# wrchen530/batrack

Measured on AMD Instinct MI355X. Metric: BA iterations/s on 64-KF/128k-edge graph, higher is better.
Workload: dtype f32

## Files before the change

### batrack_amd/csrc/ba_solve.hip

```cpp
#include <hip/hip_runtime.h>

#include "ba_kernels.hpp"
#include "ba_update.hpp"
#include "ba_wave.hpp"

namespace bt {

__device__ inline bool chol6_inv(float *Ablk, float *Linv) {
    float L[6][6];
#pragma unroll
    for (int r = 0; r < 6; ++r)
#pragma unroll
        for (int c = 0; c < 6; ++c) L[r][c] = c <= r ? Ablk[6*r + c] : 0.0f;
    bool ok = true;
#pragma unroll
    for (int c = 0; c < 6; ++c) {
        float s = L[c][c];
#pragma unroll
        for (int k = 0; k < c; ++k) s -= L[c][k] * L[c][k];
        if (!(s > 0.0f)) ok = false;
        const float l = sqrtf(s), il = 1.0f / l;
        L[c][c] = l;
#pragma unroll
        for (int r = c + 1; r < 6; ++r) {
// ... 467 lines not shown
#pragma unroll
                    for (int k = 1; k < kMaxLevelCols; ++k) q += item >= rows_before[k] ? 1 : 0;
                    const int rw = item - (q == 0 ? 0 : q == 1 ? rows_before[1] : q == 2 ? rows_before[2] : rows_before[3]);
                    const int4 ma = q == 0 ? mA0 : q == 1 ? mA1 : q == 2 ? mA2 : mA3;
                    const int j = ma.x, dpos = ma.y, cnt = ma.z;
                    T L[21];
                    const T *dblk = Lw + (size_t)dpos * 36;
#pragma unroll
                    for (int r = 0; r < 6; ++r) {
                        T row[6];
                        load_row6(dblk + 6 * r, row);
#pragma unroll
                        for (int c = 0; c <= r; ++c) L[BT_LT(r, c)] = row[c];
                    }
                    T *p = rw < cnt * 6 ? Lw + (size_t)(dpos + 1) * 36 + 6 * rw : z + 6 * j;
                    T in[6], out[6];
                    load_row6(p, in);
#pragma unroll
                    for (int c = 0; c < 6; ++c) {
                        T t = in[c];
#pragma unroll
                        for (int k = 0; k < c; ++k) t -= out[k] * L[BT_LT(c, k)];
                        out[c] = t * L[BT_LT(c, c)];
                    }
                    store_row6(p, out);
                }
            }
            BT_PF(3);
            if (PROF) { asm volatile("s_waitcnt lgkmcnt(0)" ::: "memory"); ph2 += clock64() - tph; }
            pA0 = cA0; pA1 = cA1; pA2 = cA2; pA3 = cA3; pn0 = cn0; pn1 = cn1; pn2 = cn2; pn3 = cn3;
            if (l + 1 < nlev) fetch_level(l + 1);
            __syncthreads();
            BT_PF(5);
        }

        if (PROF && lane == 0) {
            long long *o = reinterpret_cast<long long *>(a.status + 4) + 40 + wave * 2;
            o[0] = ph1; o[1] = ph2;
        }
        lds_backsub_prep<T, false>(Lw, z, zt, row_idx, col_ptr, nnzb, tid, nth);
        __syncthreads();
        BT_PF(6);
        for (int l = nlev - 1; l >= 0; --l) {
            const int4 ma = uniform4(lvl_meta[(l * kMaxLevelCols + (wave < kMaxLevelCols ? wave : 0)) * 2]);
            if (wave < kMaxLevelCols && ma.x >= 0) {
                const int c = lane >> 3, g = lane & 7;
                const int j = ma.x, dpos = ma.y, cnt = ma.z;
                T acc = (T)0;
                if (c < 6)
                    for (int sb = g; sb < cnt; sb += 8) {
                        const int b = dpos + 1 + sb;
                        T x[6];
                        load_row6(zt + 6 * (row_idx[b] & 255), x);
                        const T *mb = Lw + (size_t)b * 36 + c;
                        acc += mb[0] * x[0] + mb[6] * x[1] + mb[12] * x[2] + mb[18] * x[3] + mb[24] * x[4] + mb[30] * x[5];
                    }
                acc = dpp_add8(acc);
                if (c < 6 && g == 0) zt[6 * j + c] -= acc;
            }
            __syncthreads();
        }
        BT_PF(7);
        for (int i = tid; i < D; i += nth) if (zt[i] != zt[i]) flags[1] = 1;
        __syncthreads();
        const bool failed = flags[0] != 0, has_nan = flags[1] != 0;
        __syncthreads();
        if (failed) {
            for (int i = tid; i < D; i += nth) zt[i] = (T)0;
            status = BT_SOLVE_CHOL_FAILED;
            break;
        }
        if (!has_nan) break;
        status = BT_SOLVE_RETRIED;
    }
    __syncthreads();
    for (int i = tid; i < D; i += nth) {
        const int k = 6 * pd.perm[i / 6] + i % 6;
        a.dx[k] = (float)zt[i];
        if (PUB) dx_publish(a, k, (float)zt[i]);
    }
    if (tid == 0) a.status[0] = status;
    BT_PF(8);
    if (PROF && lane == 0 && (wave == 0 || wave == 2)) {
        long long *o = reinterpret_cast<long long *>(a.status + 4) + (wave ? 1 : 0) * 10;
        for (int i = 0; i < 10; ++i) o[i] = pf[i];
    }
#undef BT_PF
}

template <typename T, bool PROF>
__global__ __launch_bounds__(768) void k_solve_lds(PlanDev pd, StepArgs a) { solve_lds_body<T, PROF, false>(pd, a); }

template <typename T>
__device__ __forceinline__ void sys_dma_issue(const PlanDev &pd, const StepArgs &a, T *Lw, const int *bsrc, int wave, int lane, int nw) {
    static_assert(sizeof(T) == 8, "double factor");
    const int total = pd.nnzb * 18;
    const unsigned D = (unsigned)pd.D;
    for (int k = wave; k * 64 < total; k += nw) {
        const int idx = k * 64 + lane;
        if (idx < total) {
            const int b = idx / 18, rem = idx - 18 * b, r = rem / 3, h = rem - 3 * r;
            const unsigned src = (unsigned)bsrc[b], rn = src >> 9, cn = (src >> 1) & 255u;
            const double *g = a.S + ((6u * rn + (unsigned)r) * D + 6u * cn + 2u * (unsigned)h);
            __builtin_amdgcn_global_load_lds((const __attribute__((address_space(1))) void *)g,
                                             (__attribute__((address_space(3))) void *)(Lw + (size_t)k * 128), 16, 0, 0);
        }
    }
}
template <typename T>
__device__ __forceinline__ void sys_dma_fixup(const PlanDev &pd, const StepArgs &a, T *Lw, const int *trl, int ntr, const int *col_ptr, double lm, bool zero_upper, int tid, int nth) {
    for (int it = tid; it < ntr * 5; it += nth) {
        const int li = it / 5, r = it - 5 * li;
        T *blk = Lw + trl[li] * 36;
        T lo[5], up[5];
#pragma unroll
        for (int k = 0; k < 5; ++k) if (r + 1 + k < 6) { lo[k] = blk[6 * (r + 1 + k) + r]; up[k] = blk[6 * r + r + 1 + k]; }
#pragma unroll
        for (int k = 0; k < 5; ++k) if (r + 1 + k < 6) { blk[6 * (r + 1 + k) + r] = up[k]; blk[6 * r + r + 1 + k] = lo[k]; }
    }
    for (int it = tid; it < pd.D; it += nth) {
        T *dptr = Lw + col_ptr[it / 6] * 36 + 7 * (it % 6);
        const T x = *dptr;
        *dptr = x + ((T)a.ep + (T)lm * x);
    }
    if (zero_upper)
        for (int it = tid; it < pd.n * 15; it += nth) {
            const int jb = it / 15, e = it - 15 * jb, r = e >= 10 ? 5 : e >= 6 ? 4 : e >= 3 ? 3 : e >= 1 ? 2 : 1, c = e - r * (r - 1) / 2;
            Lw[col_ptr[jb] * 36 + 6 * c + r] = (T)0;
        }
}

template <typename T>
__device__ __forceinline__ void lds_load_system_dma(const PlanDev &pd, const StepArgs &a, T *Lw, T *z, int *bsrc, int *trl, int *ntr, const int *col_ptr,
                                                    double lm, bool first, bool zero_upper, int tid, int nth) {
    const int wave = tid >> 6, lane = tid & 63, nw = nth >> 6, D = pd.D;
    const int yperm = tid < D ? pd.perm[tid / 6] : 0;
    if (first) {
        if (tid == 0) *ntr = 0;
        __syncthreads();
        for (int i = tid; i < pd.nnzb; i += nth) {
            const int src = pd.blk_src[i];
            bsrc[i] = src;
            if (src & 1) trl[atomicAdd(ntr, 1)] = i;
        }
    }
    __syncthreads();
    sys_dma_issue<T>(pd, a, Lw, bsrc, wave, lane, nw);
    if (tid < D) z[tid] = (T)a.y[6 * yperm + tid % 6];
    for (int i = tid + nth; i < D; i += nth) z[i] = (T)a.y[6 * pd.perm[i / 6] + i % 6];
    __syncthreads();
    sys_dma_fixup<T>(pd, a, Lw, trl, *ntr, col_ptr, lm, zero_upper, tid, nth);
}

template <typename T, bool RAW_DIAG = false>
__device__ __forceinline__ void lds_back_substitute(const PlanDev &pd, T *Lw, T *z, T *zt, const int *row_idx,
                                                    const int *col_ptr, const int4 *lvl_meta, int mstride, int tid, int nth, long long *tprof = nullptr) {
    const int n = pd.n, nnzb = pd.nnzb, nlev = pd.nlev, wave = tid >> 6, lane = tid & 63;
    lds_backsub_prep<T, RAW_DIAG>(Lw, z, zt, row_idx, col_ptr, nnzb, tid, nth);
    __syncthreads();
    if (tprof) tprof[0] = tprof[1] = clock64();
    {
        const bool bw = wave < kMaxLevelCols;
        const int c = lane >> 3, g = lane & 7;
        struct Pre { int4 ma; int rc; T m[6]; T ztj; };
        auto preload = [&](int l, Pre &P) {
            P.ma = lvl_meta[(l * kMaxLevelCols + (bw ? wave : 0)) * mstride];
            if (!bw) P.ma.x = -1;
            if (P.ma.x >= 0 && c < 6) {
                P.ztj = zt[6 * P.ma.x + c];
                if (g < P.ma.z) {
                    const int b = P.ma.y + 1 + g;
                    P.rc = row_idx[b] & 255;
                    const T *mb = Lw + (size_t)b * 36 + c;
#pragma unroll
                    for (int k = 0; k < 6; ++k) P.m[k] = mb[6 * k];
                }
            }
        };
        auto step = [&](const Pre &P) {
            if (__builtin_amdgcn_readfirstlane(P.ma.w)) __syncthreads();
            if (P.ma.x >= 0) {
                const int j = P.ma.x, dpos = P.ma.y, cnt = P.ma.z;
                T acc = (T)0;
                if (c < 6 && g < cnt) {
                    T x[6];
                    load_row6(zt + 6 * P.rc, x);
                    acc = P.m[0] * x[0] + P.m[1] * x[1] + P.m[2] * x[2] + P.m[3] * x[3] + P.m[4] * x[4] + P.m[5] * x[5];
                    for (int sb = g + 8; sb < cnt; sb += 8) {
                        const int b = dpos + 1 + sb;
                        load_row6(zt + 6 * (row_idx[b] & 255), x);
                        const T *mb = Lw + (size_t)b * 36 + c;
                        acc += mb[0] * x[0] + mb[6] * x[1] + mb[12] * x[2] + mb[18] * x[3] + mb[24] * x[4] + mb[30] * x[5];
                    }
                }
                acc = dpp_add8(acc);
                if (c < 6 && g == 0) zt[6 * j + c] = P.ztj - acc;
                wave_fence();
            }
        };
        Pre A = {}, B = {};
        preload(nlev - 1, A);
        for (int l = nlev - 1; l >= 0; l -= 2) {
            if (l >= 1) preload(l - 1, B);
            step(A);
            if (l >= 1) {
                if (l >= 2) preload(l - 2, A);
                step(B);
            }
        }
        __syncthreads();
    }
}

template <typename T>
__device__ __forceinline__ T *row_wave_pending(T *Lw, T *z, const int *row_idx, const int *pfirst, const int *psecond, int ma, int dpos, int rw,
                                               bool &valid, T (&in)[6]) {
    const int j = ma & 255, cnt = (ma >> 8) & 255, ysrc = (ma >> 16) & 255;
    const bool isy = rw == cnt * 6;
    valid = rw <= cnt * 6;
    const int sb = rw / 6, r = rw - 6 * sb, bown = dpos + 1 + sb;
    T *p = isy ? z + 6 * j : Lw + (size_t)bown * 36 + 6 * r;
    const unsigned pfo = (unsigned)pfirst[valid && !isy ? bown : dpos];
    const int s1 = pfo & 0x7fff, s2 = (pfo >> 15) & 0x7fff, no = valid ? (int)(pfo >> 30) : 0;
    T avec[6], m[36];
    load_row6(p, in);
    load_row6(isy ? z + 6 * ysrc : Lw + (size_t)s1 * 36 + 6 * r, avec);
    {
        const T *M = Lw + (size_t)(isy ? s1 : s2) * 36;
#pragma unroll
        for (int c = 0; c < 6; ++c) load_row6(M + 6 * c, reinterpret_cast<T (&)[6]>(m[6 * c]));
    }
#pragma unroll
    for (int c = 0; c < 6; ++c) {
        T acc = avec[0] * m[6 * c];
#pragma unroll
        for (int e = 1; e < 6; ++e) acc += avec[e] * m[6 * c + e];
        in[c] -= no > 0 ? acc : (T)0;
    }
    if (__builtin_amdgcn_ballot_w64(no > 1)) {
        const unsigned ps = (unsigned)psecond[isy ? dpos : bown];
        const int t1 = ps & 0x7fff, t2 = (ps >> 15) & 0x7fff;
        load_row6(isy ? z + 6 * ((row_idx[t1] >> 8) & 255) : Lw + (size_t)t1 * 36 + 6 * r, avec);
        const T *M = Lw + (size_t)(isy ? t1 : t2) * 36;
#pragma unroll
        for (int c = 0; c < 6; ++c) load_row6(M + 6 * c, reinterpret_cast<T (&)[6]>(m[6 * c]));
#pragma unroll
        for (int c = 0; c < 6; ++c) {
            T acc = avec[0] * m[6 * c];
#pragma unroll
            for (int e = 1; e < 6; ++e) acc += avec[e] * m[6 * c + e];
            in[c] -= no > 1 ? acc : (T)0;
        }
    }
    return p;
}

__host__ __device__ inline size_t sweep_work_bytes(const PlanDev &pd) {
    const size_t b = 2 * 36 * sizeof(double) +
                     (size_t)pd.fz_nlazy * 4 * sizeof(unsigned short) + 16;
    const size_t zt = (size_t)pd.D * sizeof(double) + (size_t)pd.nlev * kMaxLevelCols * sizeof(int4);
    return ((b > zt ? b : zt) + 15) / 16 * 16;
}
size_t solve_fused_lds_bytes(const PlanDev &pd, int) {
    return ((size_t)pd.nnzb * 36 + (size_t)pd.D) * sizeof(double) + sweep_work_bytes(pd) +
           (5 * (size_t)pd.nnzb + (size_t)pd.n + 1) * sizeof(int) + 64;
}

constexpr int kFusedCols = 2;

template <bool PROF, bool PUB>
__device__ __forceinline__ void solve_fused_body(const PlanDev &pd, const StepArgs &a) {
    typedef double T;
    extern __shared__ __attribute__((aligned(16))) unsigned char smem[];
    __shared__ int flags[2];
    __shared__ int lready[kFusedCols];
    __shared__ int ntr;
    __shared__ int4 mbuf[3][2];
    const int tid = threadIdx.x, nth = blockDim.x, wave = tid >> 6, lane = tid & 63, nw = nth >> 6;
    const int n = pd.n, D = pd.D, nnzb = pd.nnzb, nlev = pd.nlev;
    T *Lw = reinterpret_cast<T *>(smem);
    T *z = Lw + (size_t)nnzb * 36, *scr = z + D, *zt = scr;
    unsigned short *lazy = reinterpret_cast<unsigned short *>(scr + kFusedCols * 36);
    int *row_idx = reinterpret_cast<int *>(reinterpret_cast<unsigned char *>(scr) + sweep_work_bytes(pd)), *pfirst = row_idx + nnzb,
        *psecond = pfirst + nnzb, *col_ptr = psecond + nnzb, *bsrc = col_ptr + n + 1, *trl = bsrc + nnzb;
    const int4 *pmeta = reinterpret_cast<const int4 *>(pd.fz_pmeta);
    for (int i = tid; i < nnzb; i += nth) { row_idx[i] = pd.fz_rowinfo[i]; pfirst[i] = pd.fz_pfirst[i]; psecond[i] = pd.fz_psecond[i]; }
    for (int i = tid; i <= n; i += nth) col_ptr[i] = pd.col_ptr[i];
    long long phA = 0, phL = 0, tph = 0, tall = PROF ? clock64() : 0, tload = 0, tsweep = 0, sub[6] = {0, 0, 0, 0, 0, 0}, tsub = 0;
#define BT_SUB(i) do { if (PROF) { asm volatile("s_waitcnt lgkmcnt(0)" ::: "memory"); const long long tq = clock64(); sub[i] += tq - tsub; tsub = tq; } } while (0)

    int status = BT_SOLVE_OK;
    for (int attempt = 0; attempt < 2; ++attempt) {
        const double lm = attempt == 0 ? 1e-4 : 1e-3;
        if (tid < 2) flags[tid] = 0;
        if (tid < kFusedCols) lready[tid] = 0;
        for (int i = tid; i < pd.fz_nlazy; i += nth)
            reinterpret_cast<ushort4 *>(lazy)[i] = make_ushort4((unsigned short)pd.fz_lazy[3 * i], (unsigned short)pd.fz_lazy[3 * i + 1],
                                                               (unsigned short)pd.fz_lazy[3 * i + 2], 0);
        if (tid < 4 && (tid >> 1) < nlev) mbuf[tid >> 1][tid & 1] = pmeta[tid];
        lds_load_system_dma<T>(pd, a, Lw, z, bsrc, trl, &ntr, col_ptr, lm, attempt == 0, true, tid, nth);
        __syncthreads();
        if (PROF) tload = clock64() - tall;

        int c0a, c0b, c0c, c0d, c1a, c1b, c1c, c1d, n0a = 0, n0b = 0, n0c = 0, n0d = 0, n1a = 0, n1b = 0, n1c = 0, n1d = 0;
        int p0a = 0, p0b = 0, p0c = 0, p1a = 0, p1b = 0, p1c = 0, pnc = 0;
        auto take_next = [&](int l) {
            const int4 m0 = mbuf[l % 3][0], m1 = mbuf[l % 3][1];
            n0a = __builtin_amdgcn_readfirstlane(m0.x); n0b = __builtin_amdgcn_readfirstlane(m0.y);
            n0c = __builtin_amdgcn_readfirstlane(m0.z); n0d = __builtin_amdgcn_readfirstlane(m0.w);
            n1a = __builtin_amdgcn_readfirstlane(m1.x); n1b = __builtin_amdgcn_readfirstlane(m1.y);
            n1c = __builtin_amdgcn_readfirstlane(m1.z); n1d = __builtin_amdgcn_readfirstlane(m1.w);
        };
        take_next(0);
        const bool feeder = tid >= nth - 2;
        for (int l = 0; l < nlev; ++l) {
            c0a = n0a; c0b = n0b; c0c = n0c; c0d = n0d; c1a = n1a; c1b = n1b; c1c = n1c; c1d = n1d;
            if (PROF) tph = clock64();
            int4 mnext = make_int4(0, 0, 0, 0);
            if (feeder && l + 2 < nlev) mnext = pmeta[(size_t)(l + 2) * 2 + (tid - (nth - 2))];
            const int cnc = (c0b >> 24) & 3;
            const int nr0 = (c0b >> 16) & 255, nr1 = cnc > 1 ? (c1b >> 16) & 255 : 0;
            const int nA = cnc + nr0 + nr1;
            for (int aw = wave; aw < nA; aw += nw) {
                __builtin_amdgcn_s_setprio(3);
                if (PROF) tsub = clock64();
                if (aw < cnc) {
                    const int q = aw, dpos = (q ? c1b : c0b) & 0xffff, md = q ? c1d : c0d;
                    const int el = lane < 36 ? lane : lane - 36, dr = el / 6, dc = el - 6 * dr;
                    const int sd = md & 0x7fff, nd = (md >> 15) & 3;
                    T x[6], yv[6];
                    T v = Lw[(size_t)dpos * 36 + el];
                    load_row6(Lw + (size_t)sd * 36 + 6 * dr, x);
                    load_row6(Lw + (size_t)sd * 36 + 6 * dc, yv);
                    if (nd > 0) {
                        T acc = x[0] * yv[0];
#pragma unroll
                        for (int e = 1; e < 6; ++e) acc += x[e] * yv[e];
                        v -= acc;
                    }
                    if (nd > 1) {
                        const T *src = Lw + (size_t)(psecond[dpos] & 0x7fff) * 36;
                        load_row6(src + 6 * dr, x);
                        load_row6(src + 6 * dc, yv);
                        T acc = x[0] * yv[0];
#pragma unroll
                        for (int e = 1; e < 6; ++e) acc += x[e] * yv[e];
                        v -= acc;
                    }
                    if (lane < 36) {
                        scr[q * 36 + lane] = v;
                        Lw[(size_t)dpos * 36 + lane] = v;
                    }
                    __builtin_amdgcn_fence(__ATOMIC_RELEASE, "workgroup");
                    if (lane == 0) __hip_atomic_store(&lready[q], l + 1, __ATOMIC_RELAXED, __HIP_MEMORY_SCOPE_WORKGROUP);
                    BT_SUB(0);
                    __builtin_amdgcn_s_setprio(0);
                } else {
                    const int ra = aw - cnc, q = ra >= nr0 ? 1 : 0, part = ra - (q ? nr0 : 0);
                    const int ma = q ? c1a : c0a, dpos = (q ? c1b : c0b) & 0xffff;
                    bool valid;
                    T in[6];
                    T *p = row_wave_pending(Lw, z, row_idx, pfirst, psecond, ma, dpos, part * 64 + lane, valid, in);
                    BT_SUB(3);
                    while (__hip_atomic_load(&lready[q], __ATOMIC_RELAXED, __HIP_MEMORY_SCOPE_WORKGROUP) <= l) __builtin_amdgcn_s_sleep(1);
                    __builtin_amdgcn_fence(__ATOMIC_ACQUIRE, "workgroup");
                    T L[21];
                    {
                        const T *dblk = scr + q * 36;
#pragma unroll
                        for (int rr = 0; rr < 6; ++rr) {
                            T row[6];
                            load_row6(dblk + 6 * rr, row);
#pragma unroll
                            for (int c = 0; c <= rr; ++c) L[BT_LT(rr, c)] = row[c];
                        }
                    }
                    const bool ok = chol6_packed<T>(L);
                    if (!ok && part == 0 && lane == 0) flags[0] = 1;
                    BT_SUB(4);
                    if (valid) {
                        T out[6];
#pragma unroll
                        for (int c = 0; c < 6; ++c) {
                            T t = in[c];
#pragma unroll
                            for (int k = 0; k < c; ++k) t -= out[k] * L[BT_LT(c, k)];
                            out[c] = t * L[BT_LT(c, c)];
                        }
                        store_row6(p, out);
                    }
                    BT_SUB(5);
                    __builtin_amdgcn_s_setprio(0);
                }
            }
            if (PROF) { asm volatile("s_waitcnt lgkmcnt(0)" ::: "memory"); const long long tn = clock64(); phA += tn - tph; tph = tn; }
            if (l > 0) {
                int h, hs;
                if (nA < nw) { h = tid - 64 * nA; hs = nth - 64 * nA; }
                else { hs = nth; h = (tid + nth - (64 * nA) % nth) % nth; }
                if (h >= 0) {
                    const int rows0 = ((p0c >> 16) & 0xffff) * 6, rows1 = rows0 + (pnc > 1 ? ((p1c >> 16) & 0xffff) * 6 : 0);
                    for (int item = h; item < rows1; item += hs) {
                        const bool sec = item >= rows0;
                        const int idx = item - (sec ? rows0 : 0), t = idx / 6;
                        const ushort4 tr = reinterpret_cast<const ushort4 *>(lazy)[((sec ? p1c : p0c) & 0xffff) + t];
                        apply_update_row3<T>(Lw, tr.x, tr.y, tr.z, idx - 6 * t);
                    }
                    {
                        const int ys0 = ((p0a >> 8) & 255) * 6, ys1 = ys0 + (pnc > 1 ? ((p1a >> 8) & 255) * 6 : 0);
                        const int shift = ((rows1 + 63) >> 6) << 6;
                        int first = h - shift;
                        if (shift > hs) first = (h - shift % hs + hs) % hs; else if (first < 0) first += hs;
                        for (int item = first; item < ys1; item += hs) {
                            const bool sec = item >= ys0;
                            const int qq = item - (sec ? ys0 : 0);
                            const int pj = (sec ? p1a : p0a) & 255, dposp = (sec ? p1b : p0b) & 0xffff, sb = qq / 6, r = qq - 6 * sb;
                            const int rcv = row_idx[dposp + 1 + sb];
                            if (rcv & (1 << 25)) continue;
                            T lr[6], zr[6];
                            load_row6(Lw + (size_t)(dposp + 1 + sb) * 36 + 6 * r, lr);
                            load_row6(z + 6 * pj, zr);
                            T acc = lr[0] * zr[0];
#pragma unroll
                            for (int k = 1; k < 6; ++k) acc += lr[k] * zr[k];
                            lds_sub(z + 6 * (rcv & 255) + r, acc, (rcv & (1 << 24)) != 0);
                        }
                    }
                }
            }
            if (feeder && l + 2 < nlev) mbuf[(l + 2) % 3][tid - (nth - 2)] = mnext;
            if (PROF) { asm volatile("s_waitcnt lgkmcnt(0)" ::: "memory"); phL += clock64() - tph; }
            p0a = c0a; p0b = c0b; p0c = c0c; p1a = c1a; p1b = c1b; p1c = c1c; pnc = cnc;
            if (l + 1 < nlev) take_next(l + 1);
            __syncthreads();
        }
        if (PROF) tsweep = clock64() - tall;

        int4 *bmeta = reinterpret_cast<int4 *>(zt + ((D + 1) & ~1));
        for (int i = tid; i < nlev * kMaxLevelCols; i += nth) {
            int4 mm = reinterpret_cast<const int4 *>(pd.fz_meta)[2 * i];
            mm.w = pd.bs_sync[i / kMaxLevelCols];
            bmeta[i] = mm;
        }
        long long tbs[2] = {0, 0};
        lds_back_substitute<T, true>(pd, Lw, z, zt, row_idx, col_ptr, bmeta, 1, tid, nth, PROF ? tbs : nullptr);
        if (PROF) { sub[0] = tbs[0] - tall; sub[1] = tbs[1] - tall; sub[2] = clock64() - tall; }
        for (int i = tid; i < D; i += nth) if (zt[i] != zt[i]) flags[1] = 1;
        __syncthreads();
        const bool failed = flags[0] != 0, has_nan = flags[1] != 0;
        __syncthreads();
        if (failed) {
            for (int i = tid; i < D; i += nth) zt[i] = (T)0;
            status = BT_SOLVE_CHOL_FAILED;
            break;
        }
        if (!has_nan) break;
        status = BT_SOLVE_RETRIED;
    }
    __syncthreads();
    for (int i = tid; i < D; i += nth) {
        const int k = 6 * pd.perm[i / 6] + i % 6;
        a.dx[k] = (float)zt[i];
        if (PUB) dx_publish(a, k, (float)zt[i]);
    }
    if (tid == 0) a.status[0] = status;
    if (PROF && lane == 0) {
        long long *o = reinterpret_cast<long long *>(a.status + 4) + 40 + wave * 2;
        o[0] = phA; o[1] = phL;
        if (wave == 0 || wave == 2) {
            long long *g = reinterpret_cast<long long *>(a.status + 4) + (wave ? 10 : 0);
            g[0] = tload; g[1] = tsweep; g[2] = clock64() - tall;
            for (int i = 0; i < 6; ++i) g[3 + i] = sub[i];
        }
    }
#undef BT_SUB
}

template <bool PROF>
__global__ __launch_bounds__(768) void k_solve_fused(PlanDev pd, StepArgs a) { solve_fused_body<PROF, false>(pd, a); }

size_t solve_pipe_lds_bytes(const PlanDev &pd) {
    return ((size_t)pd.nnzb * 36 + (size_t)pd.D) * sizeof(double) + sweep_work_bytes(pd) +
           (5 * (size_t)pd.nnzb + (size_t)pd.n + 1 + (size_t)pd.nlev * 8) * sizeof(int) + 64;
}

__device__ __forceinline__ void wait_ge(int *flag, int target) {
    while (__hip_atomic_load(flag, __ATOMIC_RELAXED, __HIP_MEMORY_SCOPE_WORKGROUP) < target) __builtin_amdgcn_s_sleep(1);
}

template <bool PROF, bool PUB>
__device__ __forceinline__ void solve_pipe_body(const PlanDev &pd, const StepArgs &a) {
    typedef double T;
    extern __shared__ __attribute__((aligned(16))) unsigned char smem[];
    __shared__ int flags[2];
    __shared__ int lready[2], colready[2], hcnt, ntr;
    const int tid = threadIdx.x, nth = blockDim.x, wave = tid >> 6, lane = tid & 63, nw = nth >> 6;
    const int n = pd.n, D = pd.D, nnzb = pd.nnzb, nlev = pd.nlev;
    T *Lw = reinterpret_cast<T *>(smem);
    T *z = Lw + (size_t)nnzb * 36, *scr = z + D, *zt = scr;
    unsigned short *lazy = reinterpret_cast<unsigned short *>(scr + 2 * 36);
    int *row_idx = reinterpret_cast<int *>(reinterpret_cast<unsigned char *>(scr) + sweep_work_bytes(pd)), *pfirst = row_idx + nnzb,
        *psecond = pfirst + nnzb, *col_ptr = psecond + nnzb, *lrec = col_ptr + n + 1, *bsrc = lrec + nlev * 8, *trl = bsrc + nnzb;
    for (int i = tid; i < nnzb; i += nth) { row_idx[i] = pd.fz_rowinfo[i]; pfirst[i] = pd.fz_pfirst[i]; psecond[i] = pd.fz_psecond[i]; }
    for (int i = tid; i <= n; i += nth) col_ptr[i] = pd.col_ptr[i];
    for (int i = tid; i < nlev * 8; i += nth) lrec[i] = pd.fz_pmeta[i];
    long long tall = PROF ? clock64() : 0, tload = 0, tsweep = 0, twait = 0, twork = 0, tq = 0, sub[3] = {0, 0, 0}, wsplit[2] = {0, 0};
#define BT_TW(acc) do { if (PROF) { asm volatile("s_waitcnt lgkmcnt(0)" ::: "memory"); const long long tn = clock64(); acc += tn - tq; tq = tn; } } while (0)

    int status = BT_SOLVE_OK;
    for (int attempt = 0; attempt < 2; ++attempt) {
        const double lm = attempt == 0 ? 1e-4 : 1e-3;
        if (tid < 2) { flags[tid] = 0; lready[tid] = 0; colready[tid] = 0; }
        if (tid == 2) hcnt = 0;
        int nlazy = pd.fz_nlazy;
        if (PUB) asm volatile("" : "+s"(nlazy));
        for (int i = tid; i < nlazy; i += nth)
            reinterpret_cast<ushort4 *>(lazy)[i] = make_ushort4((unsigned short)pd.fz_lazy[3 * i], (unsigned short)pd.fz_lazy[3 * i + 1],
                                                               (unsigned short)pd.fz_lazy[3 * i + 2], 0);
        lds_load_system_dma<T>(pd, a, Lw, z, bsrc, trl, &ntr, col_ptr, lm, attempt == 0, true, tid, nth);
        __syncthreads();
        if (PROF) { tload = clock64() - tall; tq = clock64(); }

        const int nh = nw - 4;
        if (wave < 4) {
            const int q = wave & 1;
            const bool is_row = wave >= 2;
            const int4 *lrec4 = reinterpret_cast<const int4 *>(lrec);
            int4 vrec = lrec4[q];
            int vnc = lrec[1];
            int npc = 0;
            for (int l = 0; l < nlev; ++l) {
                const int ma = __builtin_amdgcn_readfirstlane(vrec.x), mb = __builtin_amdgcn_readfirstlane(vrec.y),
                          md = __builtin_amdgcn_readfirstlane(vrec.w), ncl = (__builtin_amdgcn_readfirstlane(vnc) >> 24) & 3;
                if (l + 1 < nlev) { vrec = lrec4[2 * (l + 1) + q]; vnc = lrec[8 * (l + 1) + 1]; }
                if (q < ncl) {
                    if (l > 0) {
                        const int dep = ((md >> 20) & 3) | ((!is_row && q < npc) ? 1 << q : 0);
                        const int need0 = (dep & 1) ? l : 0, need1 = (dep & 2) ? l : 0, needh = nh * (l - 1);
                        const long long tw0 = PROF ? clock64() : 0;
                        int lastfail = -1;
                        for (;;) {
                            const int f0 = __hip_atomic_load(&colready[0], __ATOMIC_RELAXED, __HIP_MEMORY_SCOPE_WORKGROUP);
                            const int f1 = __hip_atomic_load(&colready[1], __ATOMIC_RELAXED, __HIP_MEMORY_SCOPE_WORKGROUP);
                            const int fh = __hip_atomic_load(&hcnt, __ATOMIC_RELAXED, __HIP_MEMORY_SCOPE_WORKGROUP);
                            if (f0 >= need0 && f1 >= need1 && fh >= needh) break;
                            if (PROF) lastfail = fh < needh ? 1 : 0;
                            __builtin_amdgcn_s_sleep(1);
                        }
                        if (PROF && lastfail >= 0) wsplit[lastfail] += clock64() - tw0;
                        __builtin_amdgcn_fence(__ATOMIC_ACQUIRE, "workgroup");
                    }
                    BT_TW(twait);
                    const int dpos = mb & 0xffff;
                    if (!is_row) {
                        const int el = lane < 36 ? lane : lane - 36, dr = el / 6, dc = el - 6 * dr;
                        const int sd = md & 0x7fff, nd = (md >> 15) & 3;
                        T x[6], yv[6];
                        T v = Lw[(size_t)dpos * 36 + el];
                        load_row6(Lw + (size_t)sd * 36 + 6 * dr, x);
                        load_row6(Lw + (size_t)sd * 36 + 6 * dc, yv);
                        if (nd > 0) {
                            T acc = x[0] * yv[0];
#pragma unroll
                            for (int e = 1; e < 6; ++e) acc += x[e] * yv[e];
                            v -= acc;
                        }
                        if (nd > 1) {
                            const T *src = Lw + (size_t)(psecond[dpos] & 0x7fff) * 36;
                            load_row6(src + 6 * dr, x);
                            load_row6(src + 6 * dc, yv);
                            T acc = x[0] * yv[0];
#pragma unroll
                            for (int e = 1; e < 6; ++e) acc += x[e] * yv[e];
                            v -= acc;
                        }
                        if (lane < 36) {
                            scr[q * 36 + lane] = v;
                            Lw[(size_t)dpos * 36 + lane] = v;
                        }
                        __builtin_amdgcn_fence(__ATOMIC_RELEASE, "workgroup");
                        if (lane == 0) __hip_atomic_store(&lready[q], l + 1, __ATOMIC_RELAXED, __HIP_MEMORY_SCOPE_WORKGROUP);
                        BT_TW(twork);
                    } else {
                        bool valid;
                        T in[6];
                        T *p = row_wave_pending(Lw, z, row_idx, pfirst, psecond, ma, dpos, lane, valid, in);
                        BT_TW(sub[0]);
                        wait_ge(&lready[q], l + 1);
                        __builtin_amdgcn_fence(__ATOMIC_ACQUIRE, "workgroup");
                        BT_TW(sub[1]);
                        T L[21];
                        {
                            const T *dblk = scr + q * 36;
#pragma unroll
                            for (int rr = 0; rr < 6; ++rr) {
                                T row[6];
                                load_row6(dblk + 6 * rr, row);
#pragma unroll
                                for (int c = 0; c <= rr; ++c) L[BT_LT(rr, c)] = row[c];
                            }
                        }
                        const bool ok = chol6_packed<T>(L);
                        T out[6];
#pragma unroll
                        for (int c = 0; c < 6; ++c) {
                            T t = in[c];
#pragma unroll
                            for (int k = 0; k < c; ++k) t -= out[k] * L[BT_LT(c, k)];
                            out[c] = t * L[BT_LT(c, c)];
                        }
                        if (valid) store_row6(p, out);
                        if (!ok && lane == 0) flags[0] = 1;
                        __builtin_amdgcn_fence(__ATOMIC_RELEASE, "workgroup");
                        if (lane == 0) __hip_atomic_store(&colready[q], l + 1, __ATOMIC_RELAXED, __HIP_MEMORY_SCOPE_WORKGROUP);
                        BT_TW(sub[2]);
                    }
                }
                npc = ncl;
            }
        } else {
            const int h = tid - 256, hs = nth - 256;
            for (int b = 0; b + 1 < nlev; ++b) {
                const int p0a = __builtin_amdgcn_readfirstlane(lrec[8 * b]), p0b = __builtin_amdgcn_readfirstlane(lrec[8 * b + 1]),
                          p0c = __builtin_amdgcn_readfirstlane(lrec[8 * b + 2]), p1a = __builtin_amdgcn_readfirstlane(lrec[8 * b + 4]),
                          p1b = __builtin_amdgcn_readfirstlane(lrec[8 * b + 5]), p1c = __builtin_amdgcn_readfirstlane(lrec[8 * b + 6]);
                const int pnc = (p0b >> 24) & 3;
                {
                    const int need1 = pnc > 1 ? b + 1 : 0;
                    for (;;) {
                        const int f0 = __hip_atomic_load(&colready[0], __ATOMIC_RELAXED, __HIP_MEMORY_SCOPE_WORKGROUP);
                        const int f1 = __hip_atomic_load(&colready[1], __ATOMIC_RELAXED, __HIP_MEMORY_SCOPE_WORKGROUP);
                        const int fh = __hip_atomic_load(&hcnt, __ATOMIC_RELAXED, __HIP_MEMORY_SCOPE_WORKGROUP);
                        if (f0 >= b + 1 && f1 >= need1 && fh >= nh * b) break;
                        __builtin_amdgcn_s_sleep(1);
                    }
                }
                __builtin_amdgcn_fence(__ATOMIC_ACQUIRE, "workgroup");
                BT_TW(twait);
                const int rows0 = ((p0c >> 16) & 0xffff) * 6, rows1 = rows0 + (pnc > 1 ? ((p1c >> 16) & 0xffff) * 6 : 0);
                for (int item = h; item < rows1; item += hs) {
                    const bool sec = item >= rows0;
                    const int idx = item - (sec ? rows0 : 0), t = idx / 6;
                    const ushort4 tr = reinterpret_cast<const ushort4 *>(lazy)[((sec ? p1c : p0c) & 0xffff) + t];
                    apply_update_row3<T>(Lw, tr.x, tr.y, tr.z, idx - 6 * t);
                }
                {
                    const int ys0 = ((p0a >> 8) & 255) * 6, ys1 = ys0 + (pnc > 1 ? ((p1a >> 8) & 255) * 6 : 0);
                    const int shift = ((rows1 + 63) >> 6) << 6;
                    int first = h - shift;
                    if (shift > hs) first = (h - shift % hs + hs) % hs; else if (first < 0) first += hs;
                    for (int item = first; item < ys1; item += hs) {
                        const bool sec = item >= ys0;
                        const int qq = item - (sec ? ys0 : 0);
                        const int pj = (sec ? p1a : p0a) & 255, dposp = (sec ? p1b : p0b) & 0xffff, sb = qq / 6, r = qq - 6 * sb;
                        const int rcv = row_idx[dposp + 1 + sb];
                        if (rcv & (1 << 25)) continue;
                        T lr[6], zr[6];
                        load_row6(Lw + (size_t)(dposp + 1 + sb) * 36 + 6 * r, lr);
                        load_row6(z + 6 * pj, zr);
                        T acc = lr[0] * zr[0];
#pragma unroll
                        for (int k = 1; k < 6; ++k) acc += lr[k] * zr[k];
                        lds_sub(z + 6 * (rcv & 255) + r, acc, (rcv & (1 << 24)) != 0);
                    }
                }
                __builtin_amdgcn_fence(__ATOMIC_RELEASE, "workgroup");
                if (lane == 0) __hip_atomic_fetch_add(&hcnt, 1, __ATOMIC_RELAXED, __HIP_MEMORY_SCOPE_WORKGROUP);
                BT_TW(twork);
            }
        }
        __syncthreads();
        if (PROF) tsweep = clock64() - tall;

        int4 *bmeta = reinterpret_cast<int4 *>(zt + ((D + 1) & ~1));
        for (int i = tid; i < nlev * kMaxLevelCols; i += nth) {
            int4 mm = reinterpret_cast<const int4 *>(pd.fz_meta)[2 * i];
            mm.w = pd.bs_sync[i / kMaxLevelCols];
            bmeta[i] = mm;
        }
        lds_back_substitute<T, true>(pd, Lw, z, zt, row_idx, col_ptr, bmeta, 1, tid, nth, nullptr);
        for (int i = tid; i < D; i += nth) if (zt[i] != zt[i]) flags[1] = 1;
        __syncthreads();
        const bool failed = flags[0] != 0, has_nan = flags[1] != 0;
        __syncthreads();
        if (failed) {
            for (int i = tid; i < D; i += nth) zt[i] = (T)0;
            status = BT_SOLVE_CHOL_FAILED;
            break;
        }
        if (!has_nan) break;
        status = BT_SOLVE_RETRIED;
    }
    __syncthreads();
    for (int i = tid; i < D; i += nth) {
        const int k = 6 * pd.perm[i / 6] + i % 6;
        a.dx[k] = (float)zt[i];
        if (PUB) dx_publish(a, k, (float)zt[i]);
    }
    if (tid == 0) a.status[0] = status;
    if (PROF && lane == 0) {
        long long *o = reinterpret_cast<long long *>(a.status + 4) + 40 + wave * 2;
        o[0] = twait; o[1] = twork + sub[0] + sub[2];
        if (wave == 0 || wave == 2) {
            long long *g = reinterpret_cast<long long *>(a.status + 4) + (wave ? 10 : 0);
            g[0] = tload; g[1] = tsweep; g[2] = clock64() - tall;
            g[3] = sub[0]; g[4] = sub[1]; g[5] = sub[2]; g[6] = twait; g[7] = wsplit[0]; g[8] = wsplit[1];
        }
    }
#undef BT_TW
}

template <bool PROF>
__global__ __launch_bounds__(768) void k_solve_pipe(PlanDev pd, StepArgs a) { solve_pipe_body<PROF, false>(pd, a); }

constexpr int kRefineSteps = 2;
__global__ __launch_bounds__(256) void k_refine_residual(PlanDev pd, StepArgs a, int accumulate) {
    const int D = pd.D, w = threadIdx.x >> 6, lane = threadIdx.x & 63;
    const int i = blockIdx.x * 4 + w;
    if (i >= D) return;
    const double lm = a.status[0] == BT_SOLVE_RETRIED ? 1e-3 : 1e-4;
    double acc = 0.0;
    for (int j = lane; j < D; j += 64) {
        double s = i >= j ? a.S[(size_t)i * D + j] : a.S[(size_t)j * D + i];
        if (i == j) s = s + ((double)a.ep + lm * s);
        acc += s * (double)a.dx[j];
    }
    for (int o = 32; o > 0; o >>= 1) acc += __shfl_xor(acc, o);
    if (lane == 0) a.y[i] = a.y[i] - acc;
    if (blockIdx.x == 0 && threadIdx.x < 64) {
        double nd = 0.0, nx = 0.0;
        for (int k = threadIdx.x; k < D; k += 64) {
            const float d = a.dx[k], x = accumulate ? a.dx0[k] : 0.0f;
            nd += (double)d * d; nx += (double)x * x;
            a.dx0[k] = accumulate ? x + d : d;
        }
        for (int o = 32; o > 0; o >>= 1) { nd += __shfl_xor(nd, o); nx += __shfl_xor(nx, o); }
        if (threadIdx.x == 0) a.status[kRefineDone] = (accumulate && nd <= 2.25e-8 * nx) ? 1 : 0;
    }
}

__global__ __launch_bounds__(1024) void k_refine_add(PlanDev pd, StepArgs a) {
    const bool done = a.status[kRefineDone] != 0;
    for (int k = threadIdx.x; k < pd.D; k += blockDim.x) a.dx[k] = done ? a.dx0[k] : a.dx0[k] + a.dx[k];
    __syncthreads();
    if (threadIdx.x == 0) a.status[kRefineDone] = 0;
}

Pick pick_solver(const PlanDev &pd, bool prof) {
    switch (pd.route.solver) {
    case Route::kSolvePipe:
        return prof ? pick_of<&k_solve_pipe<true>>(kSolveThreads, solve_pipe_lds_bytes(pd)) : pick_of<&k_solve_pipe<false>>(kSolveThreads, solve_pipe_lds_bytes(pd));
    case Route::kSolveFused: {
        const size_t lds = solve_fused_lds_bytes(pd, kSolveThreads);
        return prof ? pick_of<&k_solve_fused<true>>(kSolveThreads, lds) : pick_of<&k_solve_fused<false>>(kSolveThreads, lds);
    }
    case Route::kSolveLds: {
        const size_t lds = solve_lds_bytes(pd, sizeof(double));
        return prof ? pick_of<&k_solve_lds<double, true>>(kSolveThreads, lds) : pick_of<&k_solve_lds<double, false>>(kSolveThreads, lds);
    }
    case Route::kSolveLds32: {
        const size_t lds = solve_lds_bytes(pd, sizeof(float));
        return prof ? pick_of<&k_solve_lds<float, true>>(kSolveThreads, lds) : pick_of<&k_solve_lds<float, false>>(kSolveThreads, lds);
    }
    case Route::kSolveGlobal: return pick_of<&k_solve_global>(1024, 0);
    default: return Pick{};
    }
}

int launch_solve(const PlanDev &pd, const StepArgs &a, hipStream_t st, const hipEvent_t *ev) {
    const Route &r = pd.route;
    const Pick p = pick_solver(pd, (a.dbg & 16) != 0);
    const bool f32 = r.solver == Route::kSolveLds32 || r.solver == Route::kSolveGlobal;
    const int passes = f32 ? 1 + kRefineSteps : 1;
    for (int pass = 0; pass < passes; ++pass) {
        if (pass >= 1) hipLaunchKernelGGL(k_refine_residual, dim3((pd.D + 3) / 4), dim3(256), 0, st, pd, a, pass > 1 ? 1 : 0);
        launch_pick(p, 1, st, pass == 0 ? ev : nullptr, pd, a);
        if (pass >= 1 && pass == passes - 1) hipLaunchKernelGGL(k_refine_add, dim3(1), dim3(1024), 0, st, pd, a);
    }
    return hipGetLastError() == hipSuccess ? BT_OK : BT_EHIP;
}

}

#include "ba_solve_update.hpp"
```

Before: 12910.

## Precompute per-lane back-substitution table and overlap operand loads with readiness polling

Back-substitution now reads a precomputed per-lane int2 table holding column, count, block and row index, with padding levels. This removes the per-level int4 metadata decode and the row_idx lookups, and software-pipelines the operand loads for the next level ahead of the current level's accumulate. In the factor sweep, row waves issue their LDS operand loads together with the readiness-flag polls and reissue them until the flags pass. The next record and pfirst entry are also prefetched, which hides LDS latency behind the waits. This makes the memory ordering logic harder to follow and adds repeated loads while spinning.

```diff
diff --git a/batrack_amd/csrc/ba_solve.hip b/batrack_amd/csrc/ba_solve.hip
--- a/batrack_amd/csrc/ba_solve.hip
+++ b/batrack_amd/csrc/ba_solve.hip
@@ -643,84 +643,135 @@
     sys_dma_fixup<T>(pd, a, Lw, trl, *ntr, col_ptr, lm, zero_upper, tid, nth);
 }
 
+constexpr int kFusedCols = 2;
+
+constexpr int kBsSync = 1 << 16, kBsNoCol = 1 << 17, kBsNone = (int)0x80000000, kBsPad = 3;
+__host__ __device__ inline size_t backsub_table_bytes(const PlanDev &pd) { return (size_t)(pd.nlev + kBsPad) * kFusedCols * 8 * sizeof(int2); }
+__device__ __forceinline__ void backsub_table(const PlanDev &pd, int2 *tab, const int *row_idx, int tid, int nth) {
+    for (int i = tid; i < (pd.nlev + kBsPad) * kFusedCols * 8; i += nth) {
+        const int g = i & 7, ls = i >> 3, l = ls / kFusedCols - kBsPad, s = ls % kFusedCols;
+        int2 w = make_int2(kBsNoCol, kBsNone);
+        if (l >= 0) {
+            const int4 mm = reinterpret_cast<const int4 *>(pd.fz_meta)[2 * (l * kMaxLevelCols + s)];
+            const int sync = pd.bs_sync[l] ? kBsSync : 0;
+            w.x |= sync;
+            if (mm.x >= 0) {
+                const int b = mm.y + 1 + g;
+                w.x = mm.x | (mm.z << 8) | sync;
+                if (g < mm.z) w.y = b | ((row_idx[b] & 255) << 16);
+            }
+        }
+        tab[i] = w;
+    }
+}
+
 template <typename T, bool RAW_DIAG = false>
 __device__ __forceinline__ void lds_back_substitute(const PlanDev &pd, T *Lw, T *z, T *zt, const int *row_idx,
-                                                    const int *col_ptr, const int4 *lvl_meta, int mstride, int tid, int nth, long long *tprof = nullptr) {
-    const int n = pd.n, nnzb = pd.nnzb, nlev = pd.nlev, wave = tid >> 6, lane = tid & 63;
+                                                    const int *col_ptr, const int2 *tab, int tid, int nth, long long *tprof = nullptr) {
+    const int nnzb = pd.nnzb, nlev = pd.nlev, wave = tid >> 6, lane = tid & 63;
     lds_backsub_prep<T, RAW_DIAG>(Lw, z, zt, row_idx, col_ptr, nnzb, tid, nth);
     __syncthreads();
     if (tprof) tprof[0] = tprof[1] = clock64();
-    {
-        const bool bw = wave < kMaxLevelCols;
-        const int c = lane >> 3, g = lane & 7;
-        struct Pre { int4 ma; int rc; T m[6]; T ztj; };
-        auto preload = [&](int l, Pre &P) {
-            P.ma = lvl_meta[(l * kMaxLevelCols + (bw ? wave : 0)) * mstride];
-            if (!bw) P.ma.x = -1;
-            if (P.ma.x >= 0 && c < 6) {
-                P.ztj = zt[6 * P.ma.x + c];
-                if (g < P.ma.z) {
-                    const int b = P.ma.y + 1 + g;
-                    P.rc = row_idx[b] & 255;
-                    const T *mb = Lw + (size_t)b * 36 + c;
-#pragma unroll
-                    for (int k = 0; k < 6; ++k) P.m[k] = mb[6 * k];
-                }
-            }
+    const int c = lane >> 3, g = lane & 7;
+    if (__builtin_amdgcn_readfirstlane(wave) < kFusedCols) {
+        const int2 *wtab = tab + (kBsPad * kFusedCols + wave) * 8 + g;
+        struct Pre { int2 w; T m[6]; T ztj; };
+        auto word = [&](int l) { return wtab[l * (kFusedCols * 8)]; };
+        auto operands = [&](Pre &P) {
+            P.ztj = zt[6 * (P.w.x & 255) + c];
+            const T *mb = Lw + (P.w.y & 0x7fff) * 36 + c;
+#pragma unroll
+            for (int k = 0; k < 6; ++k) P.m[k] = mb[6 * k];
         };
-        auto step = [&](const Pre &P) {
-            if (__builtin_amdgcn_readfirstlane(P.ma.w)) __syncthreads();
-            if (P.ma.x >= 0) {
-                const int j = P.ma.x, dpos = P.ma.y, cnt = P.ma.z;
-                T acc = (T)0;
-                if (c < 6 && g < cnt) {
-                    T x[6];
-                    load_row6(zt + 6 * P.rc, x);
-                    acc = P.m[0] * x[0] + P.m[1] * x[1] + P.m[2] * x[2] + P.m[3] * x[3] + P.m[4] * x[4] + P.m[5] * x[5];
-                    for (int sb = g + 8; sb < cnt; sb += 8) {
-                        const int b = dpos + 1 + sb;
+        int2 wn;
+        auto level = [&](const Pre &P, Pre &N, int l2) {
+            const int wx = __builtin_amdgcn_readfirstlane(P.w.x);
+            if (wx & kBsSync) __syncthreads();
+            T x[6];
+            load_row6(zt + 6 * ((P.w.y >> 16) & 255), x);
+            __builtin_amdgcn_sched_barrier(0);
+            N.w = wn;
+            wn = word(l2);
+            operands(N);
+            __builtin_amdgcn_sched_barrier(0);
+            if (!(wx & kBsNoCol)) {
+                const int j = wx & 255, cnt = (wx >> 8) & 255;
+                T acc = P.m[0] * x[0] + P.m[1] * x[1] + P.m[2] * x[2] + P.m[3] * x[3] + P.m[4] * x[4] + P.m[5] * x[5];
+                asm volatile("" : "+v"(acc));
+                if (P.w.y < 0) acc = (T)0;
+                if (cnt > 8 && c < 6)
+                    for (int sb = g + 8, b = (P.w.y & 0x7fff) + 8; sb < cnt; sb += 8, b += 8) {
                         load_row6(zt + 6 * (row_idx[b] & 255), x);
-                        const T *mb = Lw + (size_t)b * 36 + c;
+                        const T *mb = Lw + b * 36 + c;
                         acc += mb[0] * x[0] + mb[6] * x[1] + mb[12] * x[2] + mb[18] * x[3] + mb[24] * x[4] + mb[30] * x[5];
                     }
-                }
                 acc = dpp_add8(acc);
                 if (c < 6 && g == 0) zt[6 * j + c] = P.ztj - acc;
                 wave_fence();
             }
         };
         Pre A = {}, B = {};
-        preload(nlev - 1, A);
+        A.w = word(nlev - 1);
+        wn = word(nlev - 2);
+        operands(A);
         for (int l = nlev - 1; l >= 0; l -= 2) {
-            if (l >= 1) preload(l - 1, B);
-            step(A);
-            if (l >= 1) {
-                if (l >= 2) preload(l - 2, A);
-                step(B);
-            }
-        }
-        __syncthreads();
-    }
-}
-
-template <typename T>
-__device__ __forceinline__ T *row_wave_pending(T *Lw, T *z, const int *row_idx, const int *pfirst, const int *psecond, int ma, int dpos, int rw,
-                                               bool &valid, T (&in)[6]) {
+            level(A, B, l - 2);
+            level(B, A, l - 3);
+        }
+    } else {
+        for (int l = nlev - 1; l >= 0; --l)
+            if (__builtin_amdgcn_readfirstlane(tab[(kBsPad + l) * kFusedCols * 8].x) & kBsSync) __syncthreads();
+    }
+    __syncthreads();
+}
+
+__device__ __forceinline__ int pfirst_index(int ma, int dpos, int rw) { return rw < ((ma >> 8) & 255) * 6 ? dpos + 1 + rw / 6 : dpos; }
+
+struct NoPoll {
+    __device__ __forceinline__ void look() {}
+    __device__ __forceinline__ bool passed() { return true; }
+};
+struct LevelPoll {
+    int *colready, *hcnt;
+    int need0, need1, needh, f0, f1, fh, lastfail;
+    __device__ __forceinline__ void look() {
+        f0 = __hip_atomic_load(&colready[0], __ATOMIC_RELAXED, __HIP_MEMORY_SCOPE_WORKGROUP);
+        f1 = __hip_atomic_load(&colready[1], __ATOMIC_RELAXED, __HIP_MEMORY_SCOPE_WORKGROUP);
+        fh = __hip_atomic_load(hcnt, __ATOMIC_RELAXED, __HIP_MEMORY_SCOPE_WORKGROUP);
+        asm volatile("" ::: "memory");
+    }
+    __device__ __forceinline__ bool passed() {
+        asm volatile("" ::: "memory");
+        if (f0 >= need0 && f1 >= need1 && fh >= needh) {
+            __builtin_amdgcn_fence(__ATOMIC_ACQUIRE, "workgroup");
+            return true;
+        }
+        lastfail = fh < needh ? 1 : 0;
+        __builtin_amdgcn_s_sleep(1);
+        return false;
+    }
+};
+
+template <typename T, typename Poll>
+__device__ __forceinline__ T *row_wave_pending(T *Lw, T *z, const int *row_idx, unsigned pfo, const int *psecond, int ma, int dpos, int rw,
+                                               bool &valid, T (&in)[6], Poll &poll) {
     const int j = ma & 255, cnt = (ma >> 8) & 255, ysrc = (ma >> 16) & 255;
     const bool isy = rw == cnt * 6;
     valid = rw <= cnt * 6;
     const int sb = rw / 6, r = rw - 6 * sb, bown = dpos + 1 + sb;
     T *p = isy ? z + 6 * j : Lw + (size_t)bown * 36 + 6 * r;
-    const unsigned pfo = (unsigned)pfirst[valid && !isy ? bown : dpos];
     const int s1 = pfo & 0x7fff, s2 = (pfo >> 15) & 0x7fff, no = valid ? (int)(pfo >> 30) : 0;
     T avec[6], m[36];
-    load_row6(p, in);
-    load_row6(isy ? z + 6 * ysrc : Lw + (size_t)s1 * 36 + 6 * r, avec);
-    {
-        const T *M = Lw + (size_t)(isy ? s1 : s2) * 36;
+    const T *ap = isy ? z + 6 * ysrc : Lw + (size_t)s1 * 36 + 6 * r, *M = Lw + (size_t)(isy ? s1 : s2) * 36;
+    auto look_and_load = [&]() {
+        poll.look();
+        load_row6(p, in);
+        load_row6(ap, avec);
 #pragma unroll
         for (int c = 0; c < 6; ++c) load_row6(M + 6 * c, reinterpret_cast<T (&)[6]>(m[6 * c]));
-    }
+    };
+    look_and_load();
+    while (!poll.passed()) look_and_load();
 #pragma unroll
     for (int c = 0; c < 6; ++c) {
         T acc = avec[0] * m[6 * c];
@@ -749,15 +800,13 @@
 __host__ __device__ inline size_t sweep_work_bytes(const PlanDev &pd) {
     const size_t b = 2 * 36 * sizeof(double) +
                      (size_t)pd.fz_nlazy * 4 * sizeof(unsigned short) + 16;
-    const size_t zt = (size_t)pd.D * sizeof(double) + (size_t)pd.nlev * kMaxLevelCols * sizeof(int4);
+    const size_t zt = (size_t)((pd.D + 1) & ~1) * sizeof(double) + backsub_table_bytes(pd);
     return ((b > zt ? b : zt) + 15) / 16 * 16;
 }
 size_t solve_fused_lds_bytes(const PlanDev &pd, int) {
     return ((size_t)pd.nnzb * 36 + (size_t)pd.D) * sizeof(double) + sweep_work_bytes(pd) +
            (5 * (size_t)pd.nnzb + (size_t)pd.n + 1) * sizeof(int) + 64;
 }
-
-constexpr int kFusedCols = 2;
 
 template <bool PROF, bool PUB>
 __device__ __forceinline__ void solve_fused_body(const PlanDev &pd, const StepArgs &a) {
@@ -851,7 +900,9 @@
                     const int ma = q ? c1a : c0a, dpos = (q ? c1b : c0b) & 0xffff;
                     bool valid;
                     T in[6];
-                    T *p = row_wave_pending(Lw, z, row_idx, pfirst, psecond, ma, dpos, part * 64 + lane, valid, in);
+                    NoPoll nopoll;
+                    T *p = row_wave_pending(Lw, z, row_idx, (unsigned)pfirst[pfirst_index(ma, dpos, part * 64 + lane)], psecond, ma, dpos,
+                                            part * 64 + lane, valid, in, nopoll);
                     BT_SUB(3);
                     while (__hip_atomic_load(&lready[q], __ATOMIC_RELAXED, __HIP_MEMORY_SCOPE_WORKGROUP) <= l) __builtin_amdgcn_s_sleep(1);
                     __builtin_amdgcn_fence(__ATOMIC_ACQUIRE, "workgroup");
@@ -927,14 +978,10 @@
         }
         if (PROF) tsweep = clock64() - tall;
 
-        int4 *bmeta = reinterpret_cast<int4 *>(zt + ((D + 1) & ~1));
-        for (int i = tid; i < nlev * kMaxLevelCols; i += nth) {
-            int4 mm = reinterpret_cast<const int4 *>(pd.fz_meta)[2 * i];
-            mm.w = pd.bs_sync[i / kMaxLevelCols];
-            bmeta[i] = mm;
-        }
+        int2 *btab = reinterpret_cast<int2 *>(zt + ((D + 1) & ~1));
+        backsub_table(pd, btab, row_idx, tid, nth);
         long long tbs[2] = {0, 0};
-        lds_back_substitute<T, true>(pd, Lw, z, zt, row_idx, col_ptr, bmeta, 1, tid, nth, PROF ? tbs : nullptr);
+        lds_back_substitute<T, true>(pd, Lw, z, zt, row_idx, col_ptr, btab, tid, nth, PROF ? tbs : nullptr);
         if (PROF) { sub[0] = tbs[0] - tall; sub[1] = tbs[1] - tall; sub[2] = clock64() - tall; }
         for (int i = tid; i < D; i += nth) if (zt[i] != zt[i]) flags[1] = 1;
         __syncthreads();
@@ -985,7 +1032,7 @@
     extern __shared__ __attribute__((aligned(16))) unsigned char smem[];
     __shared__ int flags[2];
     __shared__ int lready[2], colready[2], hcnt, ntr;
-    const int tid = threadIdx.x, nth = blockDim.x, wave = tid >> 6, lane = tid & 63, nw = nth >> 6;
+    const int tid = threadIdx.x, nth = blockDim.x, wave = __builtin_amdgcn_readfirstlane(tid >> 6), lane = tid & 63, nw = nth >> 6;
     const int n = pd.n, D = pd.D, nnzb = pd.nnzb, nlev = pd.nlev;
     T *Lw = reinterpret_cast<T *>(smem);
     T *z = Lw + (size_t)nnzb * 36, *scr = z + D, *zt = scr;
@@ -1004,7 +1051,7 @@
         if (tid < 2) { flags[tid] = 0; lready[tid] = 0; colready[tid] = 0; }
         if (tid == 2) hcnt = 0;
         int nlazy = pd.fz_nlazy;
-        if (PUB) asm volatile("" : "+s"(nlazy));
+        asm volatile("" : "+s"(nlazy));
         for (int i = tid; i < nlazy; i += nth)
             reinterpret_cast<ushort4 *>(lazy)[i] = make_ushort4((unsigned short)pd.fz_lazy[3 * i], (unsigned short)pd.fz_lazy[3 * i + 1],
                                                                (unsigned short)pd.fz_lazy[3 * i + 2], 0);
@@ -1020,36 +1067,28 @@
             int4 vrec = lrec4[q];
             int vnc = lrec[1];
             int npc = 0;
+            unsigned pfn = is_row ? (unsigned)pfirst[pfirst_index(vrec.x, vrec.y & 0xffff, lane)] : 0u;
             for (int l = 0; l < nlev; ++l) {
                 const int ma = __builtin_amdgcn_readfirstlane(vrec.x), mb = __builtin_amdgcn_readfirstlane(vrec.y),
                           md = __builtin_amdgcn_readfirstlane(vrec.w), ncl = (__builtin_amdgcn_readfirstlane(vnc) >> 24) & 3;
-                if (l + 1 < nlev) { vrec = lrec4[2 * (l + 1) + q]; vnc = lrec[8 * (l + 1) + 1]; }
+                auto next_record = [&]() { if (l + 1 < nlev) { vrec = lrec4[2 * (l + 1) + q]; vnc = lrec[8 * (l + 1) + 1]; } };
+                if (!is_row) next_record();
                 if (q < ncl) {
-                    if (l > 0) {
-                        const int dep = ((md >> 20) & 3) | ((!is_row && q < npc) ? 1 << q : 0);
-                        const int need0 = (dep & 1) ? l : 0, need1 = (dep & 2) ? l : 0, needh = nh * (l - 1);
-                        const long long tw0 = PROF ? clock64() : 0;
-                        int lastfail = -1;
-                        for (;;) {
-                            const int f0 = __hip_atomic_load(&colready[0], __ATOMIC_RELAXED, __HIP_MEMORY_SCOPE_WORKGROUP);
-                            const int f1 = __hip_atomic_load(&colready[1], __ATOMIC_RELAXED, __HIP_MEMORY_SCOPE_WORKGROUP);
-                            const int fh = __hip_atomic_load(&hcnt, __ATOMIC_RELAXED, __HIP_MEMORY_SCOPE_WORKGROUP);
-                            if (f0 >= need0 && f1 >= need1 && fh >= needh) break;
-                            if (PROF) lastfail = fh < needh ? 1 : 0;
-                            __builtin_amdgcn_s_sleep(1);
-                        }
-                        if (PROF && lastfail >= 0) wsplit[lastfail] += clock64() - tw0;
-                        __builtin_amdgcn_fence(__ATOMIC_ACQUIRE, "workgroup");
-                    }
-                    BT_TW(twait);
+                    const int dep = l > 0 ? ((md >> 20) & 3) | ((!is_row && q < npc) ? 1 << q : 0) : 0;
+                    LevelPoll poll = {colready, &hcnt, (dep & 1) ? l : 0, (dep & 2) ? l : 0, l > 0 ? nh * (l - 1) : 0, 0, 0, 0, -1};
+                    const long long tw0 = PROF ? clock64() : 0;
                     const int dpos = mb & 0xffff;
                     if (!is_row) {
                         const int el = lane < 36 ? lane : lane - 36, dr = el / 6, dc = el - 6 * dr;
                         const int sd = md & 0x7fff, nd = (md >> 15) & 3;
                         T x[6], yv[6];
-                        T v = Lw[(size_t)dpos * 36 + el];
+                        T v;
+                        do poll.look(); while (!poll.passed());
+                        v = Lw[(size_t)dpos * 36 + el];
                         load_row6(Lw + (size_t)sd * 36 + 6 * dr, x);
                         load_row6(Lw + (size_t)sd * 36 + 6 * dc, yv);
+                        if (PROF && poll.lastfail >= 0) wsplit[poll.lastfail] += clock64() - tw0;
+                        BT_TW(twait);
                         if (nd > 0) {
                             T acc = x[0] * yv[0];
 #pragma unroll
@@ -1075,13 +1114,14 @@
                     } else {
                         bool valid;
                         T in[6];
-                        T *p = row_wave_pending(Lw, z, row_idx, pfirst, psecond, ma, dpos, lane, valid, in);
+                        T *p = row_wave_pending(Lw, z, row_idx, pfn, psecond, ma, dpos, lane, valid, in, poll);
+                        if (PROF && poll.lastfail >= 0) wsplit[poll.lastfail] += clock64() - tw0;
                         BT_TW(sub[0]);
-                        wait_ge(&lready[q], l + 1);
-                        __builtin_amdgcn_fence(__ATOMIC_ACQUIRE, "workgroup");
-                        BT_TW(sub[1]);
                         T L[21];
-                        {
+                        int lrf;
+                        auto look_and_load = [&]() {
+                            lrf = __hip_atomic_load(&lready[q], __ATOMIC_RELAXED, __HIP_MEMORY_SCOPE_WORKGROUP);
+                            asm volatile("" ::: "memory");
                             const T *dblk = scr + q * 36;
 #pragma unroll
                             for (int rr = 0; rr < 6; ++rr) {
@@ -1090,7 +1130,14 @@
 #pragma unroll
                                 for (int c = 0; c <= rr; ++c) L[BT_LT(rr, c)] = row[c];
                             }
-                        }
+                            next_record();
+                            asm volatile("" ::: "memory");
+                        };
+                        look_and_load();
+                        while (lrf <= l) { __builtin_amdgcn_s_sleep(1); look_and_load(); }
+                        __builtin_amdgcn_fence(__ATOMIC_ACQUIRE, "workgroup");
+                        if (l + 1 < nlev) pfn = (unsigned)pfirst[pfirst_index(vrec.x, vrec.y & 0xffff, lane)];
+                        BT_TW(sub[1]);
                         const bool ok = chol6_packed<T>(L);
                         T out[6];
 #pragma unroll
@@ -1106,6 +1153,10 @@
                         if (lane == 0) __hip_atomic_store(&colready[q], l + 1, __ATOMIC_RELAXED, __HIP_MEMORY_SCOPE_WORKGROUP);
                         BT_TW(sub[2]);
                     }
+                } else if (is_row && l + 1 < nlev) {
+                    next_record();
+                    pfn = (unsigned)pfirst[pfirst_index(vrec.x, vrec.y & 0xffff, lane)];
+                    asm volatile("s_waitcnt lgkmcnt(0)" : "+v"(pfn));
                 }
                 npc = ncl;
             }
@@ -1163,13 +1214,9 @@
         __syncthreads();
         if (PROF) tsweep = clock64() - tall;
 
-        int4 *bmeta = reinterpret_cast<int4 *>(zt + ((D + 1) & ~1));
-        for (int i = tid; i < nlev * kMaxLevelCols; i += nth) {
-            int4 mm = reinterpret_cast<const int4 *>(pd.fz_meta)[2 * i];
-            mm.w = pd.bs_sync[i / kMaxLevelCols];
-            bmeta[i] = mm;
-        }
-        lds_back_substitute<T, true>(pd, Lw, z, zt, row_idx, col_ptr, bmeta, 1, tid, nth, nullptr);
+        int2 *btab = reinterpret_cast<int2 *>(zt + ((D + 1) & ~1));
+        backsub_table(pd, btab, row_idx, tid, nth);
+        lds_back_substitute<T, true>(pd, Lw, z, zt, row_idx, col_ptr, btab, tid, nth, nullptr);
         for (int i = tid; i < D; i += nth) if (zt[i] != zt[i]) flags[1] = 1;
         __syncthreads();
         const bool failed = flags[0] != 0, has_nan = flags[1] != 0;
```

Result: faster. 13350, median of 6 (+3.4%).
